# simochen/flowtrack.pytorch

Hardware: AMD Instinct MI355X
Metric: pose crops/sec (ResNet-50 + 3-deconv head, 256x192) (higher is better)
Workload: dtype fp16; 1 GPU; ResNet-50 pose head fp16, batch 64 x 256x192 synthetic crops per GPU (BASELINE.json configs[1]); per_gpu_batch=64, resident_batches=4, parallelism=dp1: batch sharded, one process per GPU

## Files before the change

flowtrack/pytorch_amd/csrc/conv_direct.hip:

```cpp
#include <stdlib.h>

#include <type_traits>

#include "ft_common.h"
#include "conv_wstat.h"

namespace ft {
namespace {

struct CdParams {
  const char* x;
  const char* x2;
  const char* res;
  char* y;
  const char* ws;
  const float* scale;
  const float* shift;
  int M;
  int nc1, nc2;
  int x_cstride, x_coff;
  int HqWq, Wq;
  int x2_hi, x2_wi, x2_cstride, x2_coff, x2_stride;
  int y_cstride, y_coff, res_cstride, res_coff;
  int Cout, act;
// ... 1135 lines not shown
  if (d->N <= 0 || d->Hi <= 0 || d->Wi <= 0) return FT_ERR_UNSUPPORTED;
  if (d->x_coff % 8 || d->x_cstride % 8 || d->y_coff % 8 || d->y_cstride % 8 || d->Cout % 64) return FT_ERR_UNSUPPORTED;
  if (d->x_cstride < d->x_coff + d->Cin || d->y_cstride < d->y_coff + d->Cout) return FT_ERR_INVALID_ARG;
  const int hw = d->Hi * d->Wi;
  if (d->stride == 2) {
    if (d->Ho != (d->Hi + 1) / 2 || d->Wo != (d->Wi + 1) / 2) return FT_ERR_UNSUPPORTED;
    if (d->Cin != 512) return FT_ERR_UNSUPPORTED;
    if (hw > 256 || d->Ho * d->Wo > 64) {
      int R = (256 / d->Wi - 1) / 2;
      if (R * d->Wo > 64) R = 64 / d->Wo;
      if (R < 1) return FT_ERR_UNSUPPORTED;
      const int nstrips = (d->Ho + R - 1) / R;
      const long long nwg = (long long)d->N * nstrips * (d->Cout / 64);
      if (nwg < 200 || nwg > 1024) return FT_ERR_UNSUPPORTED;
      if ((long long)d->N * hw * d->x_cstride * 2 >= (1LL << 31) || (long long)d->N * d->Ho * d->Wo * d->y_cstride * 2 >= (1LL << 31))
        return FT_ERR_UNSUPPORTED;
      *out = C3Plan{(R * d->Wo + 31) / 32, d->Cin / 256, 1, d->N * nstrips, d->Cout / 64, 2, R, nstrips};
      return FT_OK;
    }
    if ((long long)d->N * hw * d->x_cstride * 2 >= (1LL << 31) || (long long)d->N * d->Ho * d->Wo * d->y_cstride * 2 >= (1LL << 31))
      return FT_ERR_UNSUPPORTED;
    const int npo = d->Ho * d->Wo;
    if (2 * npo <= 96 && 2 * hw <= 512 && (long long)((d->N + 1) / 2) * (d->Cout / 64) >= 200) {
      *out = C3Plan{(2 * npo + 31) / 32, d->Cin / 256, 2, (d->N + 1) / 2, d->Cout / 64, 2};
      return FT_OK;
    }
    *out = C3Plan{(npo + 31) / 32, d->Cin / 256, 1, d->N, d->Cout / 64, 2};
    return FT_OK;
  }
  if (d->Ho != d->Hi || d->Wo != d->Wi) return FT_ERR_UNSUPPORTED;
  if (d->Cin != 512 && d->Cin != 1024) return FT_ERR_UNSUPPORTED;
  const long long M = (long long)d->N * hw;
  if (M * d->x_cstride * 2 >= (1LL << 31) || M * d->y_cstride * 2 >= (1LL << 31)) return FT_ERR_UNSUPPORTED;
  if (d->Cin == 512 && hw > 128) {
    int R = 128 / d->Wi - 2;
    if (R * d->Wi > 96) R = 96 / d->Wi;
    if (R < 2) return FT_ERR_UNSUPPORTED;
    const int nstrips = (d->Hi + R - 1) / R;
    const long long nwg = (long long)d->N * nstrips * (d->Cout / 64);
    if (nwg < 200 || nwg > 1024) return FT_ERR_UNSUPPORTED;
    *out = C3Plan{3, 2, 1, d->N * nstrips, d->Cout / 64, 1, R, nstrips};
    return FT_OK;
  }
  if (hw > (d->Cin == 512 ? 128 : 64)) return FT_ERR_UNSUPPORTED;
  const int ipw = d->Cin == 512 ? (hw <= 96 ? 96 / hw : 1) : 1;
  const int mt = d->Cin == 512 ? (ipw * hw <= 96 ? 3 : 4) : 2;
  *out = C3Plan{mt, d->Cin / 256, ipw, (d->N + ipw - 1) / ipw, d->Cout / 64, 1};
  return FT_OK;
}

template <int MT, int NLD>
static int c3s2p_launch(const C3Params& p, hipStream_t s) {
  auto k = conv3x3s2p_direct_kernel<MT, NLD>;
  constexpr int lds = 131072 + 256 + 2 * 64 * 4 + MT * 32 * 128;
  FT_RAISE_LDS(k, lds);
  hipLaunchKernelGGL(k, dim3(p.npt * p.ncb), dim3(256), lds, s, p);
  FT_LAUNCH_CHECK("conv3x3s2p_direct_kernel");
  return FT_OK;
}

template <int MT, int NH>
static int c3s2_launch(const C3Params& p, hipStream_t s) {
  auto k = conv3x3s2_direct_kernel<MT, NH>;
  constexpr int lds = 131072 + 512 + 2 * 64 * 4 + MT * 32 * 128;
  FT_RAISE_LDS(k, lds);
  hipLaunchKernelGGL(k, dim3(p.npt * p.ncb), dim3(256), lds, s, p);
  FT_LAUNCH_CHECK("conv3x3s2_direct_kernel");
  return FT_OK;
}

template <int MT, int SPT, int TT = MT>
static int c3_launch(const C3Params& p, hipStream_t s) {
  auto k = conv3x3_direct_kernel<MT, SPT, TT>;
  constexpr int lds = 131072 + SPT * 512 + 2 * 64 * 4 + MT * 32 * 128;
  static bool attr_done[64] = {};
  int dev = 0;
  FT_HIP_CHECK(hipGetDevice(&dev));
  if (dev < 0 || dev >= 64 || !attr_done[dev]) {
    FT_HIP_CHECK(hipFuncSetAttribute(reinterpret_cast<const void*>(k), hipFuncAttributeMaxDynamicSharedMemorySize, lds));
    if (dev >= 0 && dev < 64) attr_done[dev] = true;
  }
  hipLaunchKernelGGL(k, dim3(p.npt * p.ncb), dim3(256), lds, s, p);
  FT_LAUNCH_CHECK("conv3x3_direct_kernel");
  return FT_OK;
}

template <int KSPLIT>
__global__ __launch_bounds__(256) void cd_pack_kernel(const half_t* __restrict__ w, uint4_t* __restrict__ out, int nchunk, int ncb,
                                                      int kpad, int cout_pad) {
  using G = CdGeom<KSPLIT>;
  const int idx = blockIdx.x * 256 + threadIdx.x;
  const int total = ncb * nchunk * (G::WCHUNK / 16);
  if (idx >= total) return;
  const int lane = idx & 63;
  int f = idx >> 6;
  const int i = f & 1; f >>= 1;
  const int kk = f & 3; f >>= 2;
  const int wv = f & 3; f >>= 2;
  const int c = f % nchunk, cb = f / nchunk;
  const int l31 = lane & 31, lhi = lane >> 5;
  int co, k;
  if (KSPLIT == 1) {
    co = cb * 256 + (2 * wv + i) * 32 + cd_sigma(l31);
    k = c * 64 + kk * 16 + 8 * lhi;
  } else {
    co = cb * 64 + i * 32 + cd_sigma(l31);
    k = c * 256 + (4 * wv + kk) * 16 + 8 * lhi;
  }
  uint4_t v = {0u, 0u, 0u, 0u};
  if (co < cout_pad && k < kpad) v = *reinterpret_cast<const uint4_t*>(w + (size_t)co * kpad + k);
  out[idx] = v;
}


struct CsParams {
  const char* x;
  char* y;
  const char* ws;
  const float* scale;
  const float* shift;
  int M, ntiles;
  int x_cstride, x_coff, y_cstride, y_coff;
  int Cout, act;
  float slope;
  unsigned x_bytes, y_bytes, ws_bytes;
};

template <int NS, int WC, int WP, int CT, int PT>
__global__ __launch_bounds__(64 * WC * WP, 1) void conv1x1_stream_kernel(const CsParams p) {
#if defined(__HIP_DEVICE_COMPILE__)
  constexpr int NW = WC * WP, BP = WP * PT * 32, BN = WC * CT * 32, ROWB = NS * 32, SLOTB = BP * ROWB, LX = SLOTB / 1024 / NW;
  constexpr int RPL = 1024 / ROWB, CPR = ROWB / 16;
  constexpr int NST = CT * PT * 2;
  static_assert(LX * NW * 1024 == SLOTB && 2 * SLOTB <= 160 * 1024 && RPL >= 1, "shape");
  extern __shared__ __attribute__((aligned(16))) char smem[];
  typedef __attribute__((address_space(3))) void* lds_ptr;
  const int tid = threadIdx.x, lane = tid & 63;
  const int wave = __builtin_amdgcn_readfirstlane(tid >> 6);
  const int wc = wave % WC, wp = wave / WC;
  const int l31 = lane & 31, lhi = lane >> 5;
  const int cb = blockIdx.y;
  const __amdgpu_buffer_rsrc_t rsrc_x = __builtin_amdgcn_make_buffer_rsrc(const_cast<char*>(p.x), 0, p.x_bytes, 0x00020000);
  const __amdgpu_buffer_rsrc_t rsrc_y = __builtin_amdgcn_make_buffer_rsrc(p.y, 0, p.y_bytes, 0x00020000);
  const __amdgpu_buffer_rsrc_t rsrc_w = __builtin_amdgcn_make_buffer_rsrc(const_cast<char*>(p.ws), 0, p.ws_bytes, 0x00020000);
  constexpr unsigned kOOB = 0x80000000u;

  uint4_t a[CT][NS];
#pragma unroll
  for (int i = 0; i < CT; ++i)
#pragma unroll
    for (int s = 0; s < NS; ++s)
      a[i][s] = __builtin_amdgcn_raw_buffer_load_b128(rsrc_w, (unsigned)lane * 16u, ((cb * (BN / 32) + wc * CT + i) * NS + s) * 1024, 0);
  float4_t sc[CT][4], sh[CT][4];
#pragma unroll
  for (int i = 0; i < CT; ++i)
#pragma unroll
    for (int g4 = 0; g4 < 4; ++g4) {
      const int ch = cb * BN + (wc * CT + i) * 32 + 16 * lhi + 4 * g4;
      const float4_t one = {1.f, 1.f, 1.f, 1.f}, zero = {0.f, 0.f, 0.f, 0.f};
      sc[i][g4] = p.scale ? *reinterpret_cast<const float4_t*>(p.scale + ch) : one;
      sh[i][g4] = p.shift ? *reinterpret_cast<const float4_t*>(p.shift + ch) : zero;
    }
  const float act_k = p.act == FT_ACT_RELU ? 0.f : (p.act == FT_ACT_LEAKY ? p.slope : 1.f);

  int l_row[LX];
  unsigned l_off[LX];
// ... 114 lines not shown
  if ((long long)d->N * d->Hi * d->Wi * d->x_cstride * 2 >= lim || M * d->y_cstride * 2 >= lim || (d->has_residual && M * d->res_cstride * 2 >= lim) ||
      (d->x2_cin && (long long)d->N * d->x2_hi * d->x2_wi * d->x2_cstride * 2 >= lim)) return FT_ERR_UNSUPPORTED;
  static const int cs_mode = dev_env_int("FT_CD_STATIONARY", 1);
  const bool cs256 = d->Cin == 256 && d->Cout % 128 == 0 && M > 65536, cs512 = cs_mode == 2 && d->Cin == 512 && d->Cout == 256 && M >= 32768;
  if (!taps && cs_mode != 0 && !d->x2_cin && !d->has_residual && (cs256 || cs512)) {
    const int bp = cs256 ? 128 : 64;
    *out = CdPlan{0, d->Cin / 64, 0, (int)((M + bp - 1) / bp), cs256 ? d->Cout / 128 : 1};
    return FT_OK;
  }
  if (!taps && M > 65536) return FT_ERR_UNSUPPORTED;
  const int npt = (int)((M + 95) / 96);
  const bool a_ok = d->Cout % 256 == 0 && d->Cin % 64 == 0 && d->x2_cin % 64 == 0;
  const bool b_ok = d->Cin % 256 == 0 && d->x2_cin % 256 == 0;
  if (!a_ok && !b_ok) return FT_ERR_UNSUPPORTED;
  int ks = a_ok ? 1 : 4;
  if (a_ok && b_ok && (long long)npt * (d->Cout / 256) < 160 && d->Cout <= 512) ks = 4;
  const int ck = ks == 1 ? 64 : 256;
  *out = CdPlan{ks, d->kh * d->kw * (d->Cin / ck), d->x2_cin / ck, npt, d->Cout / (ks == 1 ? 256 : 64)};
  return FT_OK;
}

template <int KSPLIT, bool HAS_RES, int NCH, bool TAPS = false>
static int cd_launch(const CdParams& p, hipStream_t s) {
  auto k = conv_direct_kernel<KSPLIT, HAS_RES, NCH, TAPS>;
  constexpr int lds = CdGeom<KSPLIT>::LDS_BYTES;
  static_assert(lds <= 163840, "LDS map");
  static bool attr_done[64] = {};
  int dev = 0;
  FT_HIP_CHECK(hipGetDevice(&dev));
  if (dev < 0 || dev >= 64 || !attr_done[dev]) {
    FT_HIP_CHECK(hipFuncSetAttribute(reinterpret_cast<const void*>(k), hipFuncAttributeMaxDynamicSharedMemorySize, lds));
    if (dev >= 0 && dev < 64) attr_done[dev] = true;
  }
  hipLaunchKernelGGL(k, dim3(p.npt * p.ncb), dim3(256), lds, s, p);
  FT_LAUNCH_CHECK("conv_direct_kernel");
  return FT_OK;
}

template <int KSPLIT>
static int cd_dispatch_taps(const CdParams& p, hipStream_t s) {
  if (KSPLIT == 1) {
    switch (p.nc1) {
      case 36: return cd_launch<KSPLIT, false, 36, true>(p, s);
      case 72: return cd_launch<KSPLIT, false, 72, true>(p, s);
      default: return cd_launch<KSPLIT, false, 0, true>(p, s);
    }
  }
  switch (p.nc1) {
    case 9: return cd_launch<KSPLIT, false, 9, true>(p, s);
    case 18: return cd_launch<KSPLIT, false, 18, true>(p, s);
    default: return cd_launch<KSPLIT, false, 0, true>(p, s);
  }
}

template <int KSPLIT, bool HAS_RES>
static int cd_dispatch(const CdParams& p, hipStream_t s) {
  const int n = p.nc1 + p.nc2;
  if (KSPLIT == 1) {
    switch (n) {
      case 4: return cd_launch<KSPLIT, HAS_RES, 4>(p, s);
      case 6: return cd_launch<KSPLIT, HAS_RES, 6>(p, s);
      case 8: return cd_launch<KSPLIT, HAS_RES, 8>(p, s);
      case 12: return cd_launch<KSPLIT, HAS_RES, 12>(p, s);
      case 16: return cd_launch<KSPLIT, HAS_RES, 16>(p, s);
      case 24: return cd_launch<KSPLIT, HAS_RES, 24>(p, s);
      default: return cd_launch<KSPLIT, HAS_RES, 0>(p, s);
    }
  }
  switch (n) {
    case 2: return cd_launch<KSPLIT, HAS_RES, 2>(p, s);
    case 4: return cd_launch<KSPLIT, HAS_RES, 4>(p, s);
    case 8: return cd_launch<KSPLIT, HAS_RES, 8>(p, s);
    default: return cd_launch<KSPLIT, HAS_RES, 0>(p, s);
  }
}

}
}

extern "C" int ft_conv_direct_supported(const ft_conv_desc* d) {
  ft::CdPlan pl;
  ft::C3Plan p3;
  ft::WsPlan pw;
  if (d && d->kh == 5) return ft::ws_plan(d, &pw);
  if (d && d->kh == 3 && ft::c3_plan(d, &p3) == FT_OK) return FT_OK;
  return ft::cd_plan(d, &pl);
}

extern "C" int ft_conv_direct_stream_id(const ft_conv_desc* d) {
  ft::CdPlan pl;
  ft::C3Plan p3;
  ft::WsPlan pw;
  if (d && d->kh == 5) return ft::ws_plan(d, &pw) == FT_OK ? (0x50000000 | pw.ncg) : -1;
  if (d && d->kh == 3 && ft::c3_plan(d, &p3) == FT_OK) return 0x40000000 | (p3.stride == 2 ? (p3.ipw == 2 ? 0x30000000 : 0x10000000) : 0) | (p3.ncb << 8) | p3.spt;
  if (ft::cd_plan(d, &pl) != FT_OK) return -1;
  return ((pl.ksplit + 1) << 24) | ((pl.nc1 + pl.nc2) << 12) | pl.ncb;
}

extern "C" long long ft_conv_direct_weight_bytes(const ft_conv_desc* d) {
  ft::CdPlan pl;
  ft::C3Plan p3;
  ft::WsPlan pw;
  if (d && d->kh == 5) return ft::ws_plan(d, &pw) == FT_OK ? ft::ws_weight_bytes(pw) : 0;
  if (d && d->kh == 3 && ft::c3_plan(d, &p3) == FT_OK) return (long long)p3.ncb * 4 * 9 * p3.spt * 8192;
  if (ft::cd_plan(d, &pl) != FT_OK) return 0;
  if (pl.ksplit == 0) return (long long)d->Cout * d->Cin * 2;
  return (long long)pl.ncb * (pl.nc1 + pl.nc2) * 32768;
}

extern "C" int ft_conv_direct_pack(const ft_conv_desc* d, const void* w_packed, int kpad, int cout_pad, void* wstream, ft_stream_t stream) {
  using namespace ft;
  C3Plan p3;
  if (d && d->kh == 5) {
    WsPlan pw;
    const int st = ws_plan(d, &pw);
    return st != FT_OK ? st : ws_pack(d, pw, w_packed, kpad, cout_pad, wstream, as_stream(stream));
  }
  if (d && d->kh == 3 && c3_plan(d, &p3) == FT_OK) {
    if (!w_packed || !wstream || kpad < 9 * d->Cin || cout_pad < d->Cout) return FT_ERR_INVALID_ARG;
    const int total = p3.ncb * 4 * 9 * p3.spt * 512;
    const dim3 pg(ceil_div(total, 256));
    const half_t* wsrc = static_cast<const half_t*>(w_packed);
    uint4_t* wdst = static_cast<uint4_t*>(wstream);
    if (p3.stride == 2 && p3.ipw == 2) hipLaunchKernelGGL(c3s2p_pack_kernel, pg, dim3(256), 0, as_stream(stream), wsrc, wdst, p3.ncb, kpad, cout_pad);
    else if (p3.stride == 2) hipLaunchKernelGGL(c3s2_pack_kernel<2>, pg, dim3(256), 0, as_stream(stream), wsrc, wdst, p3.ncb, kpad, cout_pad);
    else if (p3.spt == 4) hipLaunchKernelGGL(c3_pack_kernel<4>, pg, dim3(256), 0, as_stream(stream), wsrc, wdst, p3.ncb, kpad, cout_pad);
    else hipLaunchKernelGGL(c3_pack_kernel<2>, pg, dim3(256), 0, as_stream(stream), wsrc, wdst, p3.ncb, kpad, cout_pad);
    FT_LAUNCH_CHECK("c3_pack_kernel");
    return FT_OK;
  }
  CdPlan pl;
  const int st = cd_plan(d, &pl);
  if (st != FT_OK) return st;
  if (!w_packed || !wstream || kpad < d->kh * d->kw * d->Cin + d->x2_cin || cout_pad < d->Cout) return FT_ERR_INVALID_ARG;
  const int nchunk = pl.nc1 + pl.nc2;
  const int total = pl.ncb * nchunk * 2048;
  hipStream_t s = as_stream(stream);
  if (pl.ksplit == 0) {
    const int ntile = d->Cout / 32, ns = d->Cin / 16;
    hipLaunchKernelGGL(cs_pack_kernel, dim3(ceil_div(ntile * ns * 64, 256)), dim3(256), 0, s, static_cast<const half_t*>(w_packed),
                       static_cast<uint4_t*>(wstream), ntile, ns, kpad, cout_pad);
    FT_LAUNCH_CHECK("cs_pack_kernel");
    return FT_OK;
  }
  if (pl.ksplit == 1)
    hipLaunchKernelGGL(cd_pack_kernel<1>, dim3(ceil_div(total, 256)), dim3(256), 0, s, static_cast<const half_t*>(w_packed),
                       static_cast<uint4_t*>(wstream), nchunk, pl.ncb, kpad, cout_pad);
  else
    hipLaunchKernelGGL(cd_pack_kernel<4>, dim3(ceil_div(total, 256)), dim3(256), 0, s, static_cast<const half_t*>(w_packed),
                       static_cast<uint4_t*>(wstream), nchunk, pl.ncb, kpad, cout_pad);
  FT_LAUNCH_CHECK("cd_pack_kernel");
  return FT_OK;
}

extern "C" int ft_conv_direct_fwd(const ft_conv_desc* d, const void* x, const void* wstream, const float* scale, const float* shift,
                                  const void* residual, void* y, ft_stream_t stream) {
  using namespace ft;
  C3Plan p3;
  if (d && d->kh == 5) {
    WsPlan pw;
    const int st = ws_plan(d, &pw);
    return st != FT_OK ? st : ws_launch(d, pw, x, wstream, scale, shift, y, as_stream(stream));
  }
  if (d && d->kh == 3 && c3_plan(d, &p3) == FT_OK) {
    if (!x || !wstream || !y) return FT_ERR_INVALID_ARG;
    C3Params q{};
    q.x = static_cast<const char*>(x);
    q.y = static_cast<char*>(y);
    q.ws = static_cast<const char*>(wstream);
    q.scale = scale;
    q.shift = shift;
    q.HW = d->Hi * d->Wi; q.W = d->Wi; q.H = d->Hi; q.ipw = p3.ipw;
    q.Ho = p3.stride == 2 ? d->Ho : 0; q.Wo = p3.stride == 2 ? d->Wo : 0;
    q.strip_rows = p3.strip_rows; q.nstrips = p3.nstrips;
    q.M = p3.stride == 2 ? d->N * d->Ho * d->Wo : d->N * q.HW;
    q.x_cstride = d->x_cstride; q.x_coff = d->x_coff; q.y_cstride = d->y_cstride; q.y_coff = d->y_coff;
    q.Cout = d->Cout; q.act = d->act; q.slope = d->slope;
    q.npt = p3.npt; q.ncb = p3.ncb;
    q.x_bytes = (unsigned)((size_t)d->N * q.HW * d->x_cstride * 2);
    q.y_bytes = (unsigned)((size_t)q.M * d->y_cstride * 2);
    q.ws_bytes = (unsigned)ft_conv_direct_weight_bytes(d);
    q.wmajor = cd_wmajor((long long)d->N * q.HW * d->Cin * 2, q.ws_bytes, q.npt, q.ncb);
    if (p3.stride == 2 && p3.ipw == 2) {
      const int nld = (2 * q.HW * 256 + 4095) / 4096;
      if (p3.mt <= 2) return nld <= 16 ? c3s2p_launch<2, 16>(q, as_stream(stream)) : c3s2p_launch<2, 32>(q, as_stream(stream));
      return nld <= 24 ? c3s2p_launch<3, 24>(q, as_stream(stream)) : c3s2p_launch<3, 32>(q, as_stream(stream));
    }
    if (p3.stride == 2) return p3.mt == 1 ? c3s2_launch<1, 2>(q, as_stream(stream)) : c3s2_launch<2, 2>(q, as_stream(stream));
    if (p3.strip_rows) return c3_launch<3, 2, 4>(q, as_stream(stream));
    if (p3.spt == 4) return c3_launch<2, 4>(q, as_stream(stream));
    return p3.mt == 3 ? c3_launch<3, 2>(q, as_stream(stream)) : c3_launch<4, 2>(q, as_stream(stream));
  }
  CdPlan pl;
  const int st = cd_plan(d, &pl);
  if (st != FT_OK) return st;
  if (!x || !wstream || !y || ((d->has_residual || d->x2_cin) && !residual)) return FT_ERR_INVALID_ARG;
  if (pl.ksplit == 0) {
    CsParams q{};
    q.x = static_cast<const char*>(x);
    q.y = static_cast<char*>(y);
    q.ws = static_cast<const char*>(wstream);
    q.scale = scale;
    q.shift = shift;
    q.M = d->N * d->Ho * d->Wo;
    q.ntiles = pl.npt;
    q.x_cstride = d->x_cstride; q.x_coff = d->x_coff; q.y_cstride = d->y_cstride; q.y_coff = d->y_coff;
    q.Cout = d->Cout; q.act = d->act; q.slope = d->slope;
    q.x_bytes = (unsigned)((size_t)q.M * d->x_cstride * 2);
    q.y_bytes = (unsigned)((size_t)q.M * d->y_cstride * 2);
    q.ws_bytes = (unsigned)ft_conv_direct_weight_bytes(d);
    constexpr int lds = 2 * 65536;
    int gx = 256 / pl.ncb;
    gx = gx < 1 ? 1 : (gx > pl.npt ? pl.npt : gx);
    if (d->Cin == 256) {
      auto k = conv1x1_stream_kernel<16, 2, 2, 2, 2>;
      FT_RAISE_LDS(k, lds);
      hipLaunchKernelGGL(k, dim3(gx, pl.ncb), dim3(256), lds, as_stream(stream), q);
    } else {
      auto k = conv1x1_stream_kernel<32, 8, 1, 1, 2>;
      FT_RAISE_LDS(k, lds);
      hipLaunchKernelGGL(k, dim3(gx, 1), dim3(512), lds, as_stream(stream), q);
    }
    FT_LAUNCH_CHECK("conv1x1_stream_kernel");
    return FT_OK;
  }
  CdParams p{};
  p.x = static_cast<const char*>(x);
  p.y = static_cast<char*>(y);
  p.ws = static_cast<const char*>(wstream);
  p.scale = scale;
  p.shift = shift;
  p.M = d->N * d->Ho * d->Wo;
  p.nc1 = pl.nc1; p.nc2 = pl.nc2; p.npt = pl.npt; p.ncb = pl.ncb;
  p.x_cstride = d->x_cstride; p.x_coff = d->x_coff;
  p.HqWq = d->Ho * d->Wo; p.Wq = d->Wo;
  p.y_cstride = d->y_cstride; p.y_coff = d->y_coff;
  p.Cout = d->Cout; p.act = d->act; p.slope = d->slope;
  p.x_bytes = (unsigned)((size_t)d->N * d->Hi * d->Wi * d->x_cstride * 2);
  p.y_bytes = (unsigned)((size_t)p.M * d->y_cstride * 2);
  p.ws_bytes = (unsigned)ft_conv_direct_weight_bytes(d);
  const bool taps = d->kh != 1;
// ... 21 lines not shown
```

flowtrack/pytorch_amd/hip_ops.py:

```python
from __future__ import annotations

import ctypes
import functools
import json
import os
import sys
from dataclasses import dataclass
from typing import List, Optional, Sequence, Tuple

import torch

from . import _lib
from ._lib import (FT_ACT_LEAKY, FT_ACT_NONE, FT_ACT_RELU, FT_LAYOUT_NCHW_F32, FT_LAYOUT_NHWC,
                   ConvDesc, ConvGeometry, FlowtrackHipError, check)

ACT_CODES = {None: FT_ACT_NONE, "none": FT_ACT_NONE, "relu": FT_ACT_RELU, "leaky": FT_ACT_LEAKY}


def require_gpu(device: torch.device) -> None:
    if device.type != "cuda" or not torch.cuda.is_available():
        raise FlowtrackHipError(
            "the flowtrack HIP path needs a ROCm GPU (model.cuda()); there is no CPU fallback — "
            "use oracle/ for CPU reference results")

# ... 629 lines not shown
                ch = wc * 128 + st * 16 + 4 * lhi + (e % 4) + 8 * (e // 4)
                perm = torch.stack([t[:, ch] for t in (w16, wlo)], dim=0)
                perm = perm.permute(2, 3, 0, 4, 1, 5).contiguous()
                parts.append(perm.view(torch.uint8).flatten())
            self._tail = torch.cat(parts).to(device)
            self.tail_cout = n

    def _packed_for(self, d: ConvDesc):
        key = conv_geometry(d).key()
        hit = self._packed.get(key)
        if hit is None:
            w, cout_pad = pack_conv_weights(self._weight, d, dtype=self.dtype, device=self.device)
            scale, shift = fold_scale_shift(self.cout, cout_pad, self._bias, self._bn, self.device)
            hit = self._packed[key] = (w, cout_pad, scale, shift)
        return hit

    def out_hw(self, H: int, W: int) -> Tuple[int, int]:
        if self.transposed:
            return 2 * H, 2 * W
        return (H + 2 * self.pad - self.k) // self.stride + 1, (W + 2 * self.pad - self.k) // self.stride + 1

    def record(self, prog: Program, x: ActView, y, residual: Optional[ActView] = None, pool: bool = False,
               shift_n=None, x_nchw: Optional[torch.Tensor] = None) -> None:
        if x.C != self.cin:
            raise FlowtrackHipError(f"{self.label}: input has {x.C} channels, layer expects {self.cin}")
        if x.t.dtype != self.dtype or not x.t.is_contiguous():
            raise FlowtrackHipError(f"{self.label}: input buffer must be contiguous {self.dtype}")
        if x_nchw is not None:
            if not pool or not x.rowpacked or tuple(x_nchw.shape) != (x.N, self.cin, x.H, x.W) or x_nchw.dtype != torch.float32 \
                    or not x_nchw.is_contiguous():
                raise FlowtrackHipError(f"{self.label}: x_nchw must be the contiguous fp32 [N, Cin, H, W] input of a pooled stem")
        elif x.t.device.type == "meta":
            raise FlowtrackHipError(f"{self.label}: a geometry-only input view needs x_nchw")
        Ho, Wo = self.out_hw(x.H, x.W)
        d = ConvDesc()
        d.dtype = self.code
        d.N, d.Hi, d.Wi = x.N, x.H, x.W
        d.Cin, d.x_cstride, d.x_coff = self.cin, x.cstride, x.coff
        if x.rowpacked:
            d.x_lpad, d.x_wpitch = x.lpad, x.wpitch
        d.Cout, d.kh, d.kw = self.cout, self.k, self.k
        d.stride, d.pad, d.transposed = self.stride, self.pad, int(self.transposed)
        d.Ho, d.Wo = Ho, Wo
        out_c = self.tail_cout or self.cout
        if pool:
            if Ho % 2 or Wo % 2 or not isinstance(y, ActView) or residual is not None or self.tail_cout:
                raise FlowtrackHipError(f"{self.label}: the fused max-pool needs an even conv output and a plain NHWC result")
            d.pool = 1
        yH, yW = (Ho // 2, Wo // 2) if pool else (Ho, Wo)
        if isinstance(y, ActView):
            if (y.N, y.H, y.W) != (x.N, yH, yW) or y.C != out_c or y.t.dtype != self.dtype:
                raise FlowtrackHipError(f"{self.label}: output view mismatch {tuple(y.t.shape)} C={y.C}")
            d.y_cstride, d.y_coff, d.out_layout = y.cstride, y.coff, FT_LAYOUT_NHWC
            yt = y.t
        else:
            if tuple(y.shape) != (x.N, out_c, Ho, Wo) or y.dtype != torch.float32 or not y.is_contiguous():
                raise FlowtrackHipError(f"{self.label}: NCHW output must be contiguous fp32 {(x.N, out_c, Ho, Wo)}")
            d.y_cstride, d.y_coff, d.out_layout = 0, 0, FT_LAYOUT_NCHW_F32
            yt = y
        res_ptr = None
        if residual is not None:
            if (residual.N, residual.H, residual.W) != (x.N, Ho, Wo) or residual.C != self.cout:
                raise FlowtrackHipError(f"{self.label}: residual view mismatch")
            d.has_residual, d.res_cstride, d.res_coff = 1, residual.cstride, residual.coff
            res_ptr = residual.t.data_ptr()
        d.act, d.slope = self.act, self.slope
        if self.tail_cout:
            if residual is not None:
                raise FlowtrackHipError(f"{self.label}: a fused tail excludes a residual input")
            d.tail_cout = self.tail_cout
            res_ptr = self._tail.data_ptr()
        x_ptr, x_keep = x.t.data_ptr() if x_nchw is None else x_nchw.data_ptr(), x.t if x_nchw is None else x_nchw
        if x_nchw is not None:
            d.x_nchw_f32 = 1
        w, _, scale, shift = self._packed_for(d)
        if shift_n is not None:
            d.shift_nstride = self.cout
            if self.lib.ft_conv_shift_nstride_supported(ctypes.byref(d)) != 0:
                raise FlowtrackHipError(f"{self.label}: per-sample shift is not supported for this layer / shape")
            shift = shift_n(scale, shift)
            if tuple(shift.shape) != (x.N, self.cout) or shift.dtype != torch.float32 or not shift.is_contiguous():
                raise FlowtrackHipError(f"{self.label}: per-sample shift must be contiguous fp32 {(x.N, self.cout)}")
        flops = float(self.lib.ft_conv_flops(ctypes.byref(d)))
        ws = _direct_stream(self, d, w, x.t.device) if (self.k in (1, 3, 5) and isinstance(y, ActView) and not self.tail_cout and not pool) else None
        if ws is not None:
            dd = ConvDesc.from_buffer_copy(d)
            prog.begin_choice("conv|" + _desc_key(d))
            prog.option("direct")
            prog.flops += flops
            prog.conv_records.append((self.label, len(prog.calls), flops, dd))
            prog.add("ft_conv_direct_fwd", ctypes.byref(dd), x.t.data_ptr(), ws.data_ptr(),
                     scale.data_ptr() if scale is not None else None, shift.data_ptr() if shift is not None else None, res_ptr,
                     yt.data_ptr(), keep=(dd, x.t, yt, ws, scale, shift, residual.t if residual is not None else None))
            prog.option("igemm")
        self._record_igemm(prog, d, x, w, scale, shift, res_ptr, yt, residual, flops, x_ptr, x_keep)
        if ws is not None:
            prog.end_choice()

    def _record_igemm(self, prog: Program, d: ConvDesc, x: ActView, w, scale, shift, res_ptr, yt, residual, flops: float,
                      x_ptr=None, x_keep=None) -> None:
        x_ptr = x.t.data_ptr() if x_ptr is None else x_ptr
        x_keep = x.t if x_keep is None else x_keep
        prog.flops += flops
        prog.conv_records.append((self.label, len(prog.calls), flops, d))
        if prog._side:
            prog.add("ft_conv2d_fwd", ctypes.byref(d), x_ptr, w.data_ptr(),
                     scale.data_ptr() if scale is not None else None,
                     shift.data_ptr() if shift is not None else None, res_ptr, yt.data_ptr(),
                     keep=(d, x_keep, yt, w, scale, shift, residual.t if residual is not None else None, self._tail))
            return
        prog.need_workspace(self.lib.ft_conv_workspace_bytes(ctypes.byref(d)))
        prog.add("ft_conv2d_fwd_ws", ctypes.byref(d), x_ptr, w.data_ptr(),
                 scale.data_ptr() if scale is not None else None,
                 shift.data_ptr() if shift is not None else None, res_ptr, yt.data_ptr(), prog._ws_ptr, prog._ws_size,
                 keep=(d, x_keep, yt, w, scale, shift, residual.t if residual is not None else None, self._tail))


CONV_DIRECT = os.environ.get("FT_CONV_DIRECT", "1") != "0"
CONV_DIRECT_MAX_PIXELS = int(os.environ.get("FT_CONV_DIRECT_MAX_PIXELS", "65536"))


def _direct_stream(owner, d: ConvDesc, w: torch.Tensor, device) -> Optional[torch.Tensor]:
    lib = _lib.load()
    wstat = d.kh == 5 and d.Cin == 64 and d.stride == 2 and not d.x2_cin
    if not CONV_DIRECT or d.dtype != _lib.FT_F16 or (d.Cin + d.x2_cin < 256 and not wstat) or (d.kh == 5 and not wstat):
        return None
    if not wstat and d.N * d.Ho * d.Wo > CONV_DIRECT_MAX_PIXELS and not (CONV_DIRECT_MAX_PIXELS >= 65536 and d.kh == 1 and d.Cin in (256, 512)
                                                          and not d.x2_cin and not d.has_residual):
        return None
    if lib.ft_conv_direct_supported(ctypes.byref(d)) != 0:
        return None
    sid = int(lib.ft_conv_direct_stream_id(ctypes.byref(d)))
    if sid < 0:
        return None
    key = ("direct", sid, w.data_ptr())
    hit = owner._packed.get(key)
    if hit is None:
        ws = torch.empty(int(lib.ft_conv_direct_weight_bytes(ctypes.byref(d))), dtype=torch.uint8, device=device)
        check(lib.ft_conv_direct_pack(ctypes.byref(d), w.data_ptr(), int(w.shape[-1]), int(w.shape[-2]), ws.data_ptr(),
                                      current_stream_handle(device)), "ft_conv_direct_pack")
        torch.cuda.current_stream(device).synchronize()
        hit = owner._packed[key] = ws
    return hit


class FusedShortcutConv:

    def __init__(self, w3: torch.Tensor, bn3: dict, wd: torch.Tensor, bnd: dict, stride_d: int, *, dtype: torch.dtype,
                 device: torch.device, act: Optional[str] = "relu", label: str = ""):
        require_gpu(device)
        self.lib = _lib.load()
        self.dtype, self.device, self.code = dtype, device, _lib.dtype_code(dtype)
        self.cout, self.cin = w3.shape[0], w3.shape[1]
        self.cin2, self.stride_d = wd.shape[1], stride_d
        if wd.shape[0] != self.cout or w3.shape[2:] != (1, 1) or wd.shape[2:] != (1, 1):
            raise FlowtrackHipError(f"{label}: conv3 / downsample must be 1x1 convs with the same output channels")
        self.act, self.label = ACT_CODES[act], label

        def folded(w, bn):
            s, sh = fold_scale_shift(self.cout, self.cout, None, bn, torch.device("cpu"))
            return w.detach().to(torch.float32).cpu()[:, :, 0, 0] * s[:, None], sh
        self._w3, sh3 = folded(w3, bn3)
        self._wd, shd = folded(wd, bnd)
        self._shift = sh3 + shd
        self._packed = {}

    def _packed_for(self, d: ConvDesc):
# ... 486 lines not shown
```

Before: 58970 crops/s.

## Add direct MFMA kernel for 4x4 stride-2 transposed convolutions in pose head

Adds a dedicated deconv4x4 direct kernel that decomposes the stride-2 transposed conv into four output-parity classes, keeps a whole input tile in LDS, streams pre-packed weights through registers, and fuses scale/shift/activation with a swizzled staged store. It also adds a weight-packing kernel and routes transposed k=4 layers to this path as a choice alongside implicit GEMM. The aim is to cut the im2col/igemm overhead of the deconv head layers, at the cost of a large, specialised kernel with debug/timestamp hooks and limited shape coverage.

Result: no change. 59500 crops/s (median of 6 runs) (+0.9%).

```diff
diff --git a/flowtrack/pytorch_amd/csrc/conv_direct.hip b/flowtrack/pytorch_amd/csrc/conv_direct.hip
--- a/flowtrack/pytorch_amd/csrc/conv_direct.hip
+++ b/flowtrack/pytorch_amd/csrc/conv_direct.hip
@@ -1241,6 +1241,331 @@
   }
   hipLaunchKernelGGL(k, dim3(p.npt * p.ncb), dim3(256), lds, s, p);
   FT_LAUNCH_CHECK("conv3x3_direct_kernel");
+  return FT_OK;
+}
+
+struct DcParams {
+  const char* x;
+  char* y;
+  const char* ws;
+  const float* scale;
+  const float* shift;
+  int M, HW, W, H, ipw;
+  int x_cstride, x_coff, y_cstride, y_coff;
+  int Cout, act;
+  float slope;
+  int npt, nwb;
+  unsigned x_bytes, y_bytes, ws_bytes;
+  int wmajor;
+  int dbg;
+};
+
+template <int MT, int NP>
+__global__ __launch_bounds__(256, 1) void deconv4x4_direct_kernel(const DcParams p) {
+#if defined(__HIP_DEVICE_COMPILE__)
+  constexpr int ROWB = 1024, BN = 64, NTILE = 2 * MT, SPT = 2;
+  constexpr int TROWS = MT * 32;
+  constexpr int ZROW = 131072, TAB = ZROW + ROWB, STG = TAB + 2 * BN * 4, STG_ROWB = BN * 2;
+  constexpr int PART = 4 * NTILE * 4096;
+  constexpr int NSTEP = NP * 4 * SPT;
+  static_assert(TROWS * ROWB <= ZROW && PART <= ZROW && STG + TROWS * STG_ROWB <= 163840, "LDS map");
+  extern __shared__ __attribute__((aligned(16))) char smem[];
+  using c0 = std::integral_constant<int, 0>;
+  using c1 = std::integral_constant<int, 1>;
+  const int tid = threadIdx.x, lane = tid & 63;
+  const int wave = __builtin_amdgcn_readfirstlane(tid >> 6);
+  const int l31 = lane & 31, lhi = lane >> 5;
+  int logical;
+  {
+    const int total = p.npt * p.nwb;
+    const int b = blockIdx.x;
+    const int q = total >> 3, r = total & 7, xcd = b & 7, loc = b >> 3;
+    logical = (xcd < r ? xcd * (q + 1) : r * (q + 1) + (xcd - r) * q) + loc;
+  }
+  const int wb = p.wmajor ? logical / p.npt : logical % p.nwb, pt = p.wmajor ? logical % p.npt : logical / p.nwb;
+  const int cb = wb >> 2, py = (wb >> 1) & 1, px = wb & 1;
+  const int npix = p.ipw * p.HW;
+  const int m0 = pt * npix;
+  const __amdgpu_buffer_rsrc_t rsrc_x = __builtin_amdgcn_make_buffer_rsrc(const_cast<char*>(p.x), 0, p.x_bytes, 0x00020000);
+  const __amdgpu_buffer_rsrc_t rsrc_y = __builtin_amdgcn_make_buffer_rsrc(p.y, 0, p.y_bytes, 0x00020000);
+  const __amdgpu_buffer_rsrc_t rsrc_w = __builtin_amdgcn_make_buffer_rsrc(const_cast<char*>(p.ws), 0, p.ws_bytes, 0x00020000);
+  constexpr unsigned kOOB = 0x80000000u;
+  const bool no_loads = p.dbg & 1;
+
+  constexpr int NLOAD = TROWS / 4;
+  unsigned x_voff[NLOAD];
+#pragma unroll
+  for (int t = 0; t < NLOAD; ++t) {
+    const int row = t * 4 + wave, pos = lane;
+    const int m = m0 + row;
+    x_voff[t] = (row < npix && m < p.M && !no_loads)
+                    ? (unsigned)((m * p.x_cstride + p.x_coff) * 2 + (((pos & ~15) | ((pos ^ row) & 15)) << 4)) : kOOB;
+  }
+  uint4_t treg[NLOAD];
+  auto load_tile = [&](int pass) {
+#pragma unroll
+    for (int t = 0; t < NLOAD; ++t) treg[t] = __builtin_amdgcn_raw_buffer_load_b128(rsrc_x, x_voff[t], pass * ROWB, 0);
+  };
+  auto store_tile = [&]() {
+#pragma unroll
+    for (int t = 0; t < NLOAD; ++t) *reinterpret_cast<uint4_t*>(smem + (t * 4 + wave) * 1024 + lane * 16) = treg[t];
+  };
+  const unsigned lane16 = (unsigned)lane * 16u;
+  uint4_t areg[3][4][2];
+  auto load_a = [&](auto slotc, int st) {
+    constexpr int SL = decltype(slotc)::value;
+    const int base = (st < NSTEP && !no_loads) ? ((wb * 4 + wave) * NSTEP + st) * 8192 : 0x7fff0000;
+#pragma unroll
+    for (int kk = 0; kk < 4; ++kk)
+#pragma unroll
+      for (int i = 0; i < 2; ++i)
+        areg[SL][kk][i] = __builtin_amdgcn_raw_buffer_load_b128(rsrc_w, lane16, base + (kk * 2 + i) * 1024, 0);
+  };
+  unsigned long long ts[8] = {0, 0, 0, 0, 0, 0, 0, 0};
+#define DC_TS(i) do { if (p.dbg & 32) ts[i] = __builtin_amdgcn_s_memtime(); } while (0)
+  DC_TS(0);
+  load_tile(0);
+  load_a(c0{}, 0);
+  load_a(c1{}, 1);
+  if (tid < ROWB / 16) *reinterpret_cast<uint4_t*>(smem + ZROW + tid * 16) = uint4_t{0u, 0u, 0u, 0u};
+  if (tid < BN / 4) {
+    const float4_t one = {1.f, 1.f, 1.f, 1.f}, zero = {0.f, 0.f, 0.f, 0.f};
+    const int ch = cb * BN + tid * 4;
+    reinterpret_cast<float4_t*>(smem + TAB)[tid] = p.scale ? *reinterpret_cast<const float4_t*>(p.scale + ch) : one;
+    reinterpret_cast<float4_t*>(smem + TAB + BN * 4)[tid] = p.shift ? *reinterpret_cast<const float4_t*>(p.shift + ch) : zero;
+  }
+  store_tile();
+  if constexpr (NP > 1) load_tile(1);
+  int tmask[MT];
+#pragma unroll
+  for (int j = 0; j < MT; ++j) {
+    const int pp = j * 32 + l31;
+    int mk = 0;
+    if (pp < npix) {
+      const int rem = pp % p.HW, yy = rem / p.W, xx = rem - yy * p.W;
+#pragma unroll
+      for (int t = 0; t < 4; ++t) {
+        const int ny = yy + py - (t >> 1), nx = xx + px - (t & 1);
+        if ((unsigned)ny < (unsigned)p.H && (unsigned)nx < (unsigned)p.W) mk |= 1 << t;
+      }
+    }
+    tmask[j] = mk;
+  }
+  float16_t acc[2][MT];
+#pragma unroll
+  for (int i = 0; i < 2; ++i)
+#pragma unroll
+    for (int j = 0; j < MT; ++j)
+#pragma unroll
+      for (int r = 0; r < 16; ++r) acc[i][j][r] = 0.f;
+  int rbase[4][MT];
+#pragma unroll
+  for (int t = 0; t < 4; ++t) {
+    const int off = (py - (t >> 1)) * p.W + (px - (t & 1));
+#pragma unroll
+    for (int j = 0; j < MT; ++j) {
+      const int row = j * 32 + l31 + off;
+      const int v = row * ROWB + (wave << 8) + (((lhi ^ row) & 15) << 4);
+      rbase[t][j] = ((tmask[j] >> t) & 1) ? v : ZROW + (lhi << 4);
+    }
+  }
+  uint4_t fb[2][MT];
+  auto ldb = [&](auto setc, int s, const int (&rb)[MT]) {
+    constexpr int S = decltype(setc)::value;
+#pragma unroll
+    for (int j = 0; j < MT; ++j) fb[S][j] = *reinterpret_cast<const uint4_t*>(smem + (rb[j] ^ (s << 5)));
+  };
+  auto mma = [&](auto setc, auto slotc, auto kkc) {
+    constexpr int S = decltype(setc)::value, SL = decltype(slotc)::value, kk = decltype(kkc)::value;
+#pragma unroll
+    for (int i = 0; i < 2; ++i)
+#pragma unroll
+      for (int j = 0; j < MT; ++j)
+        acc[i][j] = __builtin_amdgcn_mfma_f32_32x32x16_f16(__builtin_bit_cast(half8_t, areg[SL][kk][i]), __builtin_bit_cast(half8_t, fb[S][j]),
+                                                           acc[i][j], 0, 0, 0);
+  };
+  asm volatile("s_waitcnt lgkmcnt(0)" ::: "memory");
+  CD_BARRIER();
+  DC_TS(1);
+  ldb(c0{}, 0, rbase[0]);
+  cd_unroll<NSTEP>([&](auto sc) {
+    constexpr int st = decltype(sc)::value;
+    constexpr int pass = st / (4 * SPT), tap = (st / SPT) % 4, s0 = (st % SPT) * 4;
+    constexpr bool last_of_pass = (st + 1) % (4 * SPT) == 0;
+    using slot = std::integral_constant<int, st % 3>;
+    __builtin_amdgcn_sched_barrier(0);
+    load_a(std::integral_constant<int, (st + 2) % 3>{}, st + 2);
+    ldb(c1{}, s0 + 1, rbase[tap]);
+    __builtin_amdgcn_sched_barrier(0);
+    mma(c0{}, slot{}, std::integral_constant<int, 0>{});
+    __builtin_amdgcn_sched_barrier(0);
+    ldb(c0{}, s0 + 2, rbase[tap]);
+    __builtin_amdgcn_sched_barrier(0);
+    mma(c1{}, slot{}, std::integral_constant<int, 1>{});
+    __builtin_amdgcn_sched_barrier(0);
+    ldb(c1{}, s0 + 3, rbase[tap]);
+    __builtin_amdgcn_sched_barrier(0);
+    mma(c0{}, slot{}, std::integral_constant<int, 2>{});
+    __builtin_amdgcn_sched_barrier(0);
+    if constexpr (!last_of_pass) {
+      constexpr int ntap = ((st + 1) / SPT) % 4, ns0 = ((st + 1) % SPT) * 4;
+      ldb(c0{}, ns0, rbase[ntap]);
+      __builtin_amdgcn_sched_barrier(0);
+    }
+    mma(c1{}, slot{}, std::integral_constant<int, 3>{});
+    if constexpr (last_of_pass && st + 1 < NSTEP) {
+      __builtin_amdgcn_sched_barrier(0);
+      asm volatile("s_waitcnt lgkmcnt(0)" ::: "memory");
+      CD_BARRIER();
+      store_tile();
+      if constexpr (pass + 2 < NP) load_tile(pass + 2);
+      asm volatile("s_waitcnt lgkmcnt(0)" ::: "memory");
+      CD_BARRIER();
+      if constexpr (pass == 0) DC_TS(6);
+      if constexpr (pass == 1) DC_TS(7);
+      ldb(c0{}, 0, rbase[0]);
+    }
+  });
+  DC_TS(2);
+  asm volatile("s_waitcnt vmcnt(0) lgkmcnt(0)" ::: "memory");
+  CD_BARRIER();
+  DC_TS(3);
+
+  const float* tsc = reinterpret_cast<const float*>(smem + TAB);
+  const float* tsh = tsc + BN;
+  const float act_k = p.act == FT_ACT_RELU ? 0.f : (p.act == FT_ACT_LEAKY ? p.slope : 1.f);
+  char* stg = smem + STG;
+  float4_t* part = reinterpret_cast<float4_t*>(smem);
+#pragma unroll
+  for (int i = 0; i < 2; ++i)
+#pragma unroll
+    for (int j = 0; j < MT; ++j)
+#pragma unroll
+      for (int g4 = 0; g4 < 4; ++g4) {
+        const float4_t v = {acc[i][j][4 * g4], acc[i][j][4 * g4 + 1], acc[i][j][4 * g4 + 2], acc[i][j][4 * g4 + 3]};
+        part[((wave * NTILE + i * MT + j) * 4 + g4) * 64 + lane] = v;
+      }
+  asm volatile("s_waitcnt lgkmcnt(0)" ::: "memory");
+  CD_BARRIER();
+#pragma unroll
+  for (int k = 0; k < (NTILE + 3) / 4; ++k) {
+    const int tl = wave + 4 * k;
+    if (tl < NTILE) {
+      const int i = tl / MT, j = tl - i * MT;
+      const int ch = i * 32 + 16 * lhi, row = j * 32 + l31;
+      float4_t sc[4], sh[4];
+#pragma unroll
+      for (int g4 = 0; g4 < 4; ++g4) {
+        sc[g4] = *reinterpret_cast<const float4_t*>(tsc + ch + g4 * 4);
+        sh[g4] = *reinterpret_cast<const float4_t*>(tsh + ch + g4 * 4);
+      }
+      half8_t o[2];
+#pragma unroll
+      for (int g4 = 0; g4 < 4; ++g4) {
+        float4_t v = part[((0 * NTILE + tl) * 4 + g4) * 64 + lane];
+#pragma unroll
+        for (int w = 1; w < 4; ++w) v += part[((w * NTILE + tl) * 4 + g4) * 64 + lane];
+#pragma unroll
+        for (int e = 0; e < 4; ++e) {
+          const float u = v[e] * sc[g4][e] + sh[g4][e];
+          o[g4 >> 1][(g4 & 1) * 4 + e] = (half_t)act_mul(u, act_k);
+        }
+      }
+#pragma unroll
+      for (int h = 0; h < 2; ++h)
+        *reinterpret_cast<half8_t*>(stg + row * STG_ROWB + ((((ch >> 3) + h) ^ (row & 7)) << 4)) = o[h];
+    }
+  }
+  asm volatile("s_waitcnt lgkmcnt(0)" ::: "memory");
+  CD_BARRIER();
+  constexpr int NST = TROWS * 8 / 256;
+  const int Wo = 2 * p.W, HoWo = 4 * p.HW;
+#pragma unroll
+  for (int k = 0; k < NST; ++k) {
+    const int idx = tid + 256 * k, row = idx >> 3, ch = idx & 7;
+    const int m = m0 + row;
+    const int n = m / p.HW, rem = m - n * p.HW, yy = rem / p.W, xx = rem - yy * p.W;
+    const int mo = n * HoWo + (2 * yy + py) * Wo + 2 * xx + px;
+    const uint4_t v = *reinterpret_cast<const uint4_t*>(stg + row * STG_ROWB + ((ch ^ (row & 7)) << 4));
+    const unsigned voff = (row < npix && m < p.M && cb * BN + ch * 8 < p.Cout && !(p.dbg & 2)) ? (unsigned)((mo * p.y_cstride + p.y_coff + cb * BN + ch * 8) * 2) : kOOB;
+    __builtin_amdgcn_raw_buffer_store_b128(v, rsrc_y, voff, 0, FT_YSTORE_BUF_AUX);
+  }
+  if (p.dbg & 32) {
+    ts[4] = __builtin_amdgcn_s_memtime();
+    asm volatile("s_waitcnt vmcnt(0)" ::: "memory");
+    ts[5] = __builtin_amdgcn_s_memtime();
+    if (tid == 0 && m0 < p.M) {
+      const int n = m0 / p.HW;
+      unsigned long long* o = reinterpret_cast<unsigned long long*>(p.y + ((size_t)(n * HoWo + py * Wo + px) * p.y_cstride + p.y_coff + cb * BN) * 2);
+#pragma unroll
+      for (int i = 0; i < 8; ++i) o[i] = ts[i];
+    }
+  }
+#undef DC_TS
+#endif
+}
+
+template <int NP>
+__global__ __launch_bounds__(256) void dc_pack_kernel(const half_t* __restrict__ w, uint4_t* __restrict__ out, int ncb, int kpad, int cout_pad) {
+  constexpr int NSTEP = NP * 8;
+  const int idx = blockIdx.x * 256 + threadIdx.x;
+  if (idx >= ncb * 4 * 4 * NSTEP * 512) return;
+  const int lane = idx & 63;
+  int f = idx >> 6;
+  const int i = f & 1; f >>= 1;
+  const int kk = f & 3; f >>= 2;
+  const int st = f % NSTEP; f /= NSTEP;
+  const int wv = f & 3, wb = f >> 2;
+  const int cls = wb & 3, cb = wb >> 2;
+  const int pass = st >> 3, tap = (st >> 1) & 3, q = st & 1;
+  const int l31 = lane & 31, lhi = lane >> 5;
+  const int co = cb * 64 + i * 32 + cd_sigma(l31);
+  const int k = tap * (kpad >> 2) + pass * 512 + wv * 128 + q * 64 + kk * 16 + 8 * lhi;
+  uint4_t v = {0u, 0u, 0u, 0u};
+  if (co < cout_pad && k < kpad) v = *reinterpret_cast<const uint4_t*>(w + ((size_t)cls * cout_pad + co) * kpad + k);
+  out[idx] = v;
+}
+
+struct DcPlan {
+  int mt, np, ipw, npt, ncb;
+};
+
+static int dc_plan(const ft_conv_desc* d, DcPlan* out) {
+  if (!d) return FT_ERR_INVALID_ARG;
+  if (d->act == FT_ACT_LEAKY && !(d->slope >= 0.f && d->slope <= 1.f)) return FT_ERR_UNSUPPORTED;
+  if (d->dtype != FT_F16 || !d->transposed || d->kh != 4 || d->kw != 4 || d->stride != 2 || d->pad != 1) return FT_ERR_UNSUPPORTED;
+  if (d->tail_cout || d->pool || d->x_wpitch || d->x2_cin || d->has_residual || d->shift_nstride || d->x_nchw_f32 || d->out_layout != FT_LAYOUT_NHWC)
+    return FT_ERR_UNSUPPORTED;
+  if (d->N <= 0 || d->Hi <= 0 || d->Wi <= 0 || d->Ho != 2 * d->Hi || d->Wo != 2 * d->Wi) return FT_ERR_UNSUPPORTED;
+  if (d->x_coff % 8 || d->x_cstride % 8 || d->y_coff % 8 || d->y_cstride % 8 || d->Cout % 64) return FT_ERR_UNSUPPORTED;
+  if (d->x_cstride < d->x_coff + d->Cin || d->y_cstride < d->y_coff + d->Cout) return FT_ERR_INVALID_ARG;
+  if (d->Cin % 512 || (d->Cin != 512 && d->Cin != 2048)) return FT_ERR_UNSUPPORTED;
+  const int hw = d->Hi * d->Wi;
+  if (hw > 96) return FT_ERR_UNSUPPORTED;
+  if ((long long)d->N * hw * d->x_cstride * 2 >= (1LL << 31) || (long long)d->N * 4 * hw * d->y_cstride * 2 >= (1LL << 31)) return FT_ERR_UNSUPPORTED;
+  const int ipw = 2 * hw <= 96 ? 2 : 1;
+  const int mt = 3;
+  const int npt = (d->N + ipw - 1) / ipw, ncb = d->Cout / 64;
+  if ((long long)npt * ncb * 4 > 512) return FT_ERR_UNSUPPORTED;
+  *out = DcPlan{mt, d->Cin / 512, ipw, npt, ncb};
+  return FT_OK;
+}
+
+static inline int dc_wmajor(long long x_bytes, long long w_bytes, int npt, int nwb) {
+  static const int mode = dev_env_int("FT_DC_WMAJOR", 0);
+  if (mode != 2) return mode == 1;
+  if (nwb < 8 || npt < 2) return 0;
+  return 8 * x_bytes + w_bytes < x_bytes + 8 * w_bytes;
+}
+
+template <int MT, int NP>
+static int dc_launch(const DcParams& p, hipStream_t s) {
+  auto k = deconv4x4_direct_kernel<MT, NP>;
+  constexpr int lds = 131072 + 1024 + 2 * 64 * 4 + MT * 32 * 128;
+  static_assert(lds <= 163840, "LDS map");
+  FT_RAISE_LDS(k, lds);
+  hipLaunchKernelGGL(k, dim3(p.npt * p.nwb), dim3(256), lds, s, p);
+  FT_LAUNCH_CHECK("deconv4x4_direct_kernel");
   return FT_OK;
 }
 
@@ -1521,6 +1846,8 @@
   ft::CdPlan pl;
   ft::C3Plan p3;
   ft::WsPlan pw;
+  ft::DcPlan pd;
+  if (d && d->transposed) return ft::dc_plan(d, &pd);
   if (d && d->kh == 5) return ft::ws_plan(d, &pw);
   if (d && d->kh == 3 && ft::c3_plan(d, &p3) == FT_OK) return FT_OK;
   return ft::cd_plan(d, &pl);
@@ -1530,6 +1857,8 @@
   ft::CdPlan pl;
   ft::C3Plan p3;
   ft::WsPlan pw;
+  ft::DcPlan pd;
+  if (d && d->transposed) return ft::dc_plan(d, &pd) == FT_OK ? (0x60000000 | (pd.ncb << 8) | pd.np) : -1;
   if (d && d->kh == 5) return ft::ws_plan(d, &pw) == FT_OK ? (0x50000000 | pw.ncg) : -1;
   if (d && d->kh == 3 && ft::c3_plan(d, &p3) == FT_OK) return 0x40000000 | (p3.stride == 2 ? (p3.ipw == 2 ? 0x30000000 : 0x10000000) : 0) | (p3.ncb << 8) | p3.spt;
   if (ft::cd_plan(d, &pl) != FT_OK) return -1;
@@ -1540,6 +1869,8 @@
   ft::CdPlan pl;
   ft::C3Plan p3;
   ft::WsPlan pw;
+  ft::DcPlan pd;
+  if (d && d->transposed) return ft::dc_plan(d, &pd) == FT_OK ? (long long)pd.ncb * 4 * 4 * 8 * pd.np * 8192 : 0;
   if (d && d->kh == 5) return ft::ws_plan(d, &pw) == FT_OK ? ft::ws_weight_bytes(pw) : 0;
   if (d && d->kh == 3 && ft::c3_plan(d, &p3) == FT_OK) return (long long)p3.ncb * 4 * 9 * p3.spt * 8192;
   if (ft::cd_plan(d, &pl) != FT_OK) return 0;
@@ -1550,6 +1881,20 @@
 extern "C" int ft_conv_direct_pack(const ft_conv_desc* d, const void* w_packed, int kpad, int cout_pad, void* wstream, ft_stream_t stream) {
   using namespace ft;
   C3Plan p3;
+  if (d && d->transposed) {
+    DcPlan pd;
+    const int st = dc_plan(d, &pd);
+    if (st != FT_OK) return st;
+    if (!w_packed || !wstream || kpad != 4 * d->Cin || cout_pad < d->Cout) return FT_ERR_INVALID_ARG;
+    const int total = pd.ncb * 4 * 4 * 8 * pd.np * 512;
+    const dim3 pg(ceil_div(total, 256));
+    const half_t* wsrc = static_cast<const half_t*>(w_packed);
+    uint4_t* wdst = static_cast<uint4_t*>(wstream);
+    if (pd.np == 4) hipLaunchKernelGGL(dc_pack_kernel<4>, pg, dim3(256), 0, as_stream(stream), wsrc, wdst, pd.ncb, kpad, cout_pad);
+    else hipLaunchKernelGGL(dc_pack_kernel<1>, pg, dim3(256), 0, as_stream(stream), wsrc, wdst, pd.ncb, kpad, cout_pad);
+    FT_LAUNCH_CHECK("dc_pack_kernel");
+    return FT_OK;
+  }
   if (d && d->kh == 5) {
     WsPlan pw;
     const int st = ws_plan(d, &pw);
@@ -1596,6 +1941,30 @@
                                   const void* residual, void* y, ft_stream_t stream) {
   using namespace ft;
   C3Plan p3;
+  if (d && d->transposed) {
+    DcPlan pd;
+    const int st = dc_plan(d, &pd);
+    if (st != FT_OK) return st;
+    if (!x || !wstream || !y) return FT_ERR_INVALID_ARG;
+    DcParams q{};
+    q.x = static_cast<const char*>(x);
+    q.y = static_cast<char*>(y);
+    q.ws = static_cast<const char*>(wstream);
+    q.scale = scale;
+    q.shift = shift;
+    q.HW = d->Hi * d->Wi; q.W = d->Wi; q.H = d->Hi; q.ipw = pd.ipw;
+    q.M = d->N * q.HW;
+    q.x_cstride = d->x_cstride; q.x_coff = d->x_coff; q.y_cstride = d->y_cstride; q.y_coff = d->y_coff;
+    q.Cout = d->Cout; q.act = d->act; q.slope = d->slope;
+    q.npt = pd.npt; q.nwb = pd.ncb * 4;
+    q.x_bytes = (unsigned)((size_t)q.M * d->x_cstride * 2);
+    q.y_bytes = (unsigned)((size_t)q.M * 4 * d->y_cstride * 2);
+    q.ws_bytes = (unsigned)ft_conv_direct_weight_bytes(d);
+    q.wmajor = dc_wmajor((long long)q.M * d->Cin * 2, q.ws_bytes, q.npt, q.nwb);
+    static const int dc_dbg = dev_env_int("FT_DC_DBG", 0);
+    q.dbg = dc_dbg;
+    return pd.np == 4 ? dc_launch<3, 4>(q, as_stream(stream)) : dc_launch<3, 1>(q, as_stream(stream));
+  }
   if (d && d->kh == 5) {
     WsPlan pw;
     const int st = ws_plan(d, &pw);
diff --git a/flowtrack/pytorch_amd/hip_ops.py b/flowtrack/pytorch_amd/hip_ops.py
--- a/flowtrack/pytorch_amd/hip_ops.py
+++ b/flowtrack/pytorch_amd/hip_ops.py
@@ -735,7 +735,7 @@
             if tuple(shift.shape) != (x.N, self.cout) or shift.dtype != torch.float32 or not shift.is_contiguous():
                 raise FlowtrackHipError(f"{self.label}: per-sample shift must be contiguous fp32 {(x.N, self.cout)}")
         flops = float(self.lib.ft_conv_flops(ctypes.byref(d)))
-        ws = _direct_stream(self, d, w, x.t.device) if (self.k in (1, 3, 5) and isinstance(y, ActView) and not self.tail_cout and not pool) else None
+        ws = _direct_stream(self, d, w, x.t.device) if ((self.k in (1, 3, 5) or (self.transposed and self.k == 4)) and isinstance(y, ActView) and not self.tail_cout and not pool) else None
         if ws is not None:
             dd = ConvDesc.from_buffer_copy(d)
             prog.begin_choice("conv|" + _desc_key(d))
```
